# localdevices/pyorc

Measured on AMD Instinct MI355X. Metric: PIV frame-pairs/sec, 1080p 32x32@50% overlap (Mvectors/sec in config), higher is better.
Workload: dtype f32; 1 GPU; synthetic 1080x1920 uint8 particle stack, 1000 frame-pairs per GPU, 32x32 windows @ overlap 16 (BASELINE.json configs[1]); frame_dtype=u8, windows_per_pair=7854, parallelism=single GPU

## Files before the change

### pyorc_amd/csrc/api_internal.h

```cpp
#pragma once

#include "../../include/lspiv.h"

#include <hip/hip_runtime.h>

#include <atomic>
#include <cstdint>
#include <mutex>
#include <vector>

#include "common.h"
#include "host_stage.h"

namespace lspiv_api __attribute__((visibility("hidden"))) {

int fail(int code, const char* fmt, ...);

inline int hip_code(hipError_t e) {
  return e == hipErrorOutOfMemory ? LSPIV_ENOMEM : (e == hipErrorNoDevice || e == hipErrorNoBinaryForGpu) ? LSPIV_ENODEV : LSPIV_EHIP;
}

#define HIP_TRY(expr)                                                                                          \
  do {                                                                                                         \
    const hipError_t e_ = (expr);                                                                              \
    if (e_ != hipSuccess)                                                                                      \
      return fail(hip_code(e_), "%s failed: %s (%s:%d)", #expr, hipGetErrorString(e_), __FILE__, __LINE__);    \
  } while (0)

#define LSPIV_TRY(expr)                                                                        \
  do {                                                                                         \
    const int rc_ = (expr);                                                                    \
    if (rc_ != LSPIV_OK) return rc_;                                                           \
  } while (0)

inline int launch_status(hipError_t e, const char* what = "kernel launch failed", int oom_code = LSPIV_EHIP) {
  if (e == hipSuccess) return LSPIV_OK;
  return fail(e == hipErrorOutOfMemory ? oom_code : LSPIV_EHIP, "%s: %s", what, hipGetErrorString(e));
}

inline size_t elem_size(int dtype) { return dtype == LSPIV_U8 ? 1 : dtype == LSPIV_F32 ? 4 : 8; }

struct Grid {
  int64_t n_rows = 0, n_cols = 0;
};
int make_grid(int64_t H, int64_t W, int wy, int wx, int oy, int ox, Grid* g);

struct DeviceCtx {
  hipStream_t stream = nullptr;
  hipStream_t copy_stream = nullptr;
  void* d_frames = nullptr;  size_t frames_cap = 0;
  float* d_out = nullptr;    size_t out_cap = 0;
  float* d_planes = nullptr; size_t planes_cap = 0;
  void* d_scratch = nullptr; size_t scratch_cap = 0;
  void* d_dft = nullptr; size_t dft_cap = 0;
  uint8_t* d_keep = nullptr; size_t keep_cap = 0;
  struct RescueWs { hipStream_t stream; void* base; size_t cap_bytes; uint32_t cap_fit, cap_amb; };
  std::vector<RescueWs> rescue;
  void* pinned[2] = {nullptr, nullptr}; size_t pinned_cap = 0;
  hipEvent_t staged[2] = {nullptr, nullptr};
  struct ProjWs { hipStream_t stream = nullptr; void* d_in = nullptr; size_t in_cap = 0; void* d_out = nullptr; size_t out_cap = 0;
                  void* pin[2] = {nullptr, nullptr}; hipEvent_t ev[2] = {nullptr, nullptr}; };
  static constexpr size_t kProjPinBytes = (size_t)16 << 20;
  static constexpr int kProjSlots = 2;
  ProjWs proj[kProjSlots];
  bool arch_ok = false;
};
constexpr int kMaxDevices = 64;
struct DeviceLocks { std::mutex host, dispatch, lists, project[DeviceCtx::kProjSlots]; std::atomic<unsigned> next_project{0}; };
extern DeviceLocks g_locks[kMaxDevices];
int current_device_slot();
inline DeviceLocks& locks_here() { return g_locks[current_device_slot()]; }
int get_ctx(DeviceCtx** out);
inline hipStream_t on_stream(const DeviceCtx* c, void* stream) { return stream ? (hipStream_t)stream : c->stream; }
template <class Launch>
int launch_on(void* stream, Launch&& launch) {
  DeviceCtx* c;
  const int rc = get_ctx(&c);
  return rc ? rc : launch_status(launch(on_stream(c, stream)));
}

struct TraceRec { int kind; hipEvent_t e0, e1; };
struct Trace;
struct TraceSpan {
  Trace* t = nullptr; TraceRec r{};
  ~TraceSpan();
};
void trace_begin(TraceSpan* sp, int kind, hipStream_t s);
void trace_end(TraceSpan* sp, hipStream_t s);

// ... 73 lines not shown
```

### pyorc_amd/csrc/api_piv.hip

```cpp
#include "api_internal.h"

#include <algorithm>
#include <cmath>
#include <cstdlib>
#include <cstring>

namespace lspiv_api __attribute__((visibility("hidden"))) {

int check_window(int wy, int wx, int oy, int ox) {
  if (wy < 2 || wx < 2 || wy > LSPIV_MAX_WINDOW || wx > LSPIV_MAX_WINDOW)
    return fail(LSPIV_EUNSUPPORTED, "window %dx%d outside supported range 2..%d", wy, wx, LSPIV_MAX_WINDOW);
  if (oy < 0 || ox < 0 || oy >= wy || ox >= wx)
    return fail(LSPIV_EINVAL, "overlap (%d,%d) must satisfy 0 <= overlap < window (%d,%d)", oy, ox, wy, wx);
  return LSPIV_OK;
}

int64_t axis_shape(int64_t dim, int win, int ov) { return dim < win ? 0 : (dim - win) / (win - ov) + 1; }

int make_grid(int64_t H, int64_t W, int wy, int wx, int oy, int ox, Grid* g) {
  LSPIV_TRY(check_window(wy, wx, oy, ox));
  if (H <= 0 || W <= 0) return fail(LSPIV_ESHAPE, "frame shape (%lld,%lld) invalid", (long long)H, (long long)W);
  g->n_rows = axis_shape(H, wy, oy);
  g->n_cols = axis_shape(W, wx, ox);
  if (g->n_rows <= 0 || g->n_cols <= 0)
    return fail(LSPIV_ESHAPE, "frame (%lld,%lld) smaller than window (%d,%d)", (long long)H, (long long)W, wy, wx);
  return LSPIV_OK;
}

int rescue_ws(DeviceCtx* c, hipStream_t s, uint32_t n_tiles, lspiv::PivParams* p) {
  std::lock_guard<std::mutex> lk(locks_here().lists);
  DeviceCtx::RescueWs* ws = nullptr;
  for (auto& w : c->rescue) if (w.stream == s) ws = &w;
  if (!ws) { c->rescue.push_back({s, nullptr, 0, 0, 0}); ws = &c->rescue.back(); }
  const uint32_t cap_fit = std::max<uint32_t>(4096u, n_tiles / 4u), cap_amb = std::max<uint32_t>(1024u, n_tiles / 16u);
  const size_t hdr_bytes = 256;
  static_assert(sizeof(lspiv::RescueHdr) <= 256, "header slot too small");
  if (cap_fit > ws->cap_fit || cap_amb > ws->cap_amb || !ws->base) {
    const uint32_t nf = std::max(cap_fit, ws->cap_fit), na = std::max(cap_amb, ws->cap_amb);
    const size_t bytes = hdr_bytes + (size_t)nf * sizeof(uint4) + (size_t)na * sizeof(uint32_t);
    void* grown = nullptr;
    HIP_TRY(hipMalloc(&grown, bytes));
    if (ws->base) {
      hipError_t e = hipStreamSynchronize(s);
      if (e == hipSuccess) e = hipMemcpy(grown, ws->base, hdr_bytes, hipMemcpyDeviceToDevice);
      if (e != hipSuccess) { (void)hipFree(grown); return fail(LSPIV_EHIP, "rescue lists: %s", hipGetErrorString(e)); }
      HIP_TRY(hipFree(ws->base));
    } else {
      HIP_TRY(hipMemsetAsync(grown, 0, hdr_bytes, s));
    }
    ws->base = grown;
    ws->cap_bytes = bytes; ws->cap_fit = nf; ws->cap_amb = na;
  }
  p->rescue_hdr = static_cast<lspiv::RescueHdr*>(ws->base);
  p->rescue_fit = reinterpret_cast<uint4*>((char*)ws->base + hdr_bytes);
  p->rescue_amb = reinterpret_cast<uint32_t*>((char*)ws->base + hdr_bytes + (size_t)ws->cap_fit * sizeof(uint4));
  p->rescue_cap_fit = ws->cap_fit;
  p->rescue_cap_amb = ws->cap_amb;
  return LSPIV_OK;
}

int fill_params(lspiv::PivParams* p, const void* d_frames, int dtype, int64_t T, int64_t H, int64_t W, int wy, int wx,
                int oy, int ox, float signal_threshold, const Grid& g) {
  if (dtype < 0 || dtype > 2) return fail(LSPIV_EINVAL, "dtype %d not in {0:u8, 1:f32, 2:f64}", dtype);
  if (T < 2) return fail(LSPIV_ESHAPE, "need at least 2 frames, got %lld", (long long)T);
  const int64_t n_win = g.n_rows * g.n_cols;
  const int64_t n_tiles = (T - 1) * n_win;
  if (n_tiles >= (int64_t)1 << 31 || H * W >= (int64_t)1 << 31)
    return fail(LSPIV_EINVAL, "chunk too large for one launch: %lld windows (limit 2^31); use smaller chunks",
                (long long)n_tiles);
  memset(p, 0, sizeof(*p));
  p->frames = d_frames;
  p->frame_elems = H * W;
  p->H = (int)H; p->W = (int)W;
  p->wy = wy; p->wx = wx;
  p->sy = wy - oy; p->sx = wx - ox;
  p->n_rows = (int)g.n_rows; p->n_cols = (int)g.n_cols;
  p->n_win = (uint32_t)n_win;
  p->n_tiles = (uint32_t)n_tiles;
  p->n_pairs = (uint32_t)(T - 1);
  p->signal_threshold = signal_threshold;
  p->border_mode = g_opt_border.load();
  p->nz_positive = g_opt_signal_pos.load();
  {
    const double n = (double)wy * (double)wx;
    const double g2 = g_opt_std_ddof.load() && n > 1.0 ? (n - 1.0) / n : 1.0;
    p->std_gain2 = (float)g2;
// ... 4 lines not shown
  p->rescue_tau = (float)(g_opt_rescue_tau.load() * 1e-9);
  p->div_ncols = lspiv::FastDiv::make((uint32_t)g.n_cols);
  p->div_jobs = lspiv::FastDiv::make((uint32_t)((n_win + 1) / 2));
  p->div_nwin = lspiv::FastDiv::make((uint32_t)n_win);
  return LSPIV_OK;
}

static int dispatch_kernels(const lspiv::PivParams& p, int dtype, bool ensemble, hipStream_t s);

constexpr int kTimerRing = 16;
struct KernelTimer { hipEvent_t e0[kTimerRing] = {}, e1[kTimerRing] = {}; int n = 0; };
KernelTimer g_timers[kMaxDevices];
static int timed_dispatch_kernels(const lspiv::PivParams& p, int dtype, bool ensemble, hipStream_t s) {
  if (!g_opt_time_kernel.load()) return dispatch_kernels(p, dtype, ensemble, s);
  KernelTimer& t = g_timers[current_device_slot()];
  const int k = t.n % kTimerRing;
  if (!t.e0[k]) { HIP_TRY(hipEventCreate(&t.e0[k])); HIP_TRY(hipEventCreate(&t.e1[k])); }
  HIP_TRY(hipEventRecord(t.e0[k], s));
  LSPIV_TRY(dispatch_kernels(p, dtype, ensemble, s));
  HIP_TRY(hipEventRecord(t.e1[k], s));
  ++t.n;
  return LSPIV_OK;
}
int dispatch(const lspiv::PivParams& p0, int dtype, bool ensemble, hipStream_t s) {
  if (ensemble || !g_opt_rescue.load()) {
    if (!g_opt_time_kernel.load()) return dispatch_kernels(p0, dtype, ensemble, s);
    std::lock_guard<std::mutex> launch_lock(locks_here().dispatch);
    return timed_dispatch_kernels(p0, dtype, ensemble, s);
  }
  DeviceCtx* c;
  LSPIV_TRY(get_ctx(&c));
  lspiv::PivParams p = p0;
  std::lock_guard<std::mutex> launch_lock(locks_here().dispatch);
  LSPIV_TRY(rescue_ws(c, s, p.n_tiles, &p));
  LSPIV_TRY(timed_dispatch_kernels(p, dtype, false, s));
  return launch_status(lspiv::launch_piv_rescue(p, dtype, s), "rescue kernel launch failed");
}

int apply_v_sign(float* d_v, int64_t n, hipStream_t s) {
  if (!g_opt_v_sign.load() || !d_v) return LSPIV_OK;
  return launch_status(lspiv::launch_negate(d_v, n, s));
}

static int dispatch_kernels(const lspiv::PivParams& p, int dtype, bool ensemble, hipStream_t s) {
  const int kind = lspiv_kernel_kind(p.wy, p.wx);
  hipError_t e;
  switch (kind) {
    case 7: e = lspiv::launch_piv_embed16(p, dtype, ensemble, s); break;
    case 4: e = lspiv::launch_piv_embed32(p, dtype, ensemble, s); break;
    case 5: e = lspiv::launch_piv_embed64(p, dtype, ensemble, s); break;
    case 6: e = p.wy == 8 ? lspiv::launch_piv_fft8(p, dtype, ensemble, s) : lspiv::launch_piv_fft16(p, dtype, ensemble, s); break;
    case 8:
      switch (p.wy) {
#define LSPIV_PFA_CASE(n) case n: e = lspiv::launch_piv_fft##n(p, dtype, ensemble, s); break;
        LSPIV_PFA_SIZES(LSPIV_PFA_CASE)
#undef LSPIV_PFA_CASE
        default: return fail(LSPIV_EUNSUPPORTED, "no prime-factor kernel for window %d", p.wy);
      }
      break;
    case 1: e = lspiv::launch_piv_fft32(p, dtype, ensemble, s); break;
    case 2: e = lspiv::launch_piv_fft64(p, dtype, ensemble, s); break;
    case 3: e = lspiv::launch_piv_direct(p, dtype, ensemble, s); break;
    case 9: e = lspiv::launch_piv_dft(p, dtype, ensemble, s); break;
    case 10: {
      DeviceCtx* c;
      LSPIV_TRY(get_ctx(&c));
      const size_t slot = lspiv::piv_dft_global_slot_floats(p.wy, p.wx);
      const int blocks = lspiv::piv_dft_global_blocks(ensemble ? p.n_win : p.n_tiles);
      LSPIV_TRY(ensure(&c->d_dft, &c->dft_cap, slot * (size_t)blocks * sizeof(float)));
// ... 310 lines not shown
```

### pyorc_amd/csrc/common.h

```cpp
#pragma once
#include <hip/hip_runtime.h>
#include <stdint.h>

#include <algorithm>

namespace lspiv {

struct FastDiv {
  uint32_t magic, shift, d;
  static __host__ FastDiv make(uint32_t d) {
    FastDiv f;
    f.d = d;
    uint32_t l = 31;
    while (l > 0 && !((d >> l) & 1u)) --l;
    if ((d & (d - 1)) == 0) {
      f.magic = 0;
      f.shift = l == 0 ? 0 : l - 1;
      return f;
    }
    const uint64_t num = (uint64_t)1 << (32 + l);
    uint64_t m = num / d;
    const uint64_t rem = num - m * d;
    m += m;
    const uint64_t twice_rem = rem + rem;
    if (twice_rem >= d) m += 1;
    f.magic = (uint32_t)(m + 1);
    f.shift = l;
    return f;
  }
  __host__ __device__ __forceinline__ uint32_t div(uint32_t n) const {
    if (d == 1) return n;
#ifdef __HIP_DEVICE_COMPILE__
    const uint32_t q = __umulhi(magic, n);
#else
    const uint32_t q = (uint32_t)(((uint64_t)magic * n) >> 32);
#endif
    return (((n - q) >> 1) + q) >> shift;
  }
};

struct RescueHdr {
  uint32_t n_fit, n_amb;
  uint32_t spare0, spare1;
  uint32_t done_blocks, pad;
  uint32_t last_fit, last_amb;
  unsigned long long total_fit, total_amb, total_windows;
};

struct PivParams {
  const void* frames;
  int64_t frame_elems;
  int H, W;
  int wy, wx;
  int sy, sx;
  int n_rows, n_cols;
  uint32_t n_win;
  uint32_t n_tiles;
  float signal_threshold;
  int border_mode;
  int nz_positive;
  const uint8_t* win_keep;
  float std_gain, std_gain2;
  int norm_clip;
  float* u;
  float* v;
  float* cmax;
  float* s2n;
  float* planes;
  float corr_min, s2n_min;
  float* corr_sum;
  float* corr_count;
  float* part_sum;
  float* part_cnt;
  float* dft_scratch;
  size_t dft_slot;
  uint32_t seg_len, n_seg;
  uint32_t seg_first;
// ... 215 lines not shown
__device__ __forceinline__ void rescue_note(RescueHdr* hdr, uint4* fit, uint32_t cap_fit, uint32_t* amb, uint32_t cap_amb,
                                            uint32_t g, PeakCond c, int ip, int jp, uint32_t pos2 = 0xffffffffu) {
  if (c.amb && pos2 == 0xffffffffu) {
    const uint32_t i = atomicAdd(&hdr->n_amb, 1u);
    if (i < cap_amb) amb[i] = g;
  } else if (c.amb || c.fit) {
    const uint32_t i = atomicAdd(&hdr->n_fit, 1u);
    if (i < cap_fit) fit[i] = make_uint4(g, ((uint32_t)ip << 16) | (uint32_t)jp, pos2, 0u);
  }
}

__device__ __forceinline__ float to_f32(uint8_t x) { return (float)x; }
__device__ __forceinline__ float to_f32(float x) { return x; }
__device__ __forceinline__ float to_f32(double x) { return (float)x; }

hipError_t launch_piv_fft8(const PivParams& p, int dtype, bool ensemble, hipStream_t s);
hipError_t launch_piv_fft16(const PivParams& p, int dtype, bool ensemble, hipStream_t s);
#define LSPIV_PFA_SIZES(X) X(6) X(10) X(12) X(14) X(18) X(20) X(22) X(24) X(26) X(28) X(30) X(34) X(36) X(38) X(40) X(42) X(44) X(46) \
  X(48) X(50) X(52) X(54) X(56) X(58) X(60) X(62)
#define LSPIV_PFA_DECL(n) hipError_t launch_piv_fft##n(const PivParams& p, int dtype, bool ensemble, hipStream_t s);
LSPIV_PFA_SIZES(LSPIV_PFA_DECL)
#undef LSPIV_PFA_DECL
hipError_t launch_piv_fft32(const PivParams& p, int dtype, bool ensemble, hipStream_t s);
hipError_t launch_piv_fft64(const PivParams& p, int dtype, bool ensemble, hipStream_t s);
hipError_t launch_piv_direct(const PivParams& p, int dtype, bool ensemble, hipStream_t s);
hipError_t launch_piv_dft(const PivParams& p, int dtype, bool ensemble, hipStream_t s);
bool piv_dft_fits(int wy, int wx);
size_t piv_dft_global_slot_floats(int wy, int wx);
int piv_dft_global_blocks(uint32_t n_work);
hipError_t launch_piv_dft_global(const PivParams& p, int dtype, bool ensemble, hipStream_t s);
hipError_t launch_piv_embed16(const PivParams& p, int dtype, bool ensemble, hipStream_t s);
hipError_t launch_piv_embed32(const PivParams& p, int dtype, bool ensemble, hipStream_t s);
hipError_t launch_piv_embed64(const PivParams& p, int dtype, bool ensemble, hipStream_t s);
hipError_t launch_piv_rescue(const PivParams& p, int dtype, hipStream_t s);
hipError_t launch_ens_flag(const float* mean, uint32_t n_win, int wy, int wx, const float* u, const float* v, float k, float tau,
                           EnsRescueHdr* hdr, EnsRescueRec* recs, uint32_t cap, hipStream_t s);
hipError_t launch_ens_partial(const PivParams& p, int dtype, const EnsRescueArgs& a, hipStream_t s);
hipError_t launch_ens_merge(const EnsRescueArgs& a, double* totals, hipStream_t s);
hipError_t launch_ens_final(const PivParams& p, const EnsRescueArgs& a, const double* totals, float* u, float* v, hipStream_t s);
hipError_t launch_peaks_from_planes(const float* planes, uint32_t n_planes, int wy, int wx, int border_mode,
                                    float* u, float* v, hipStream_t s);
hipError_t launch_window_signal(const void* frames, int dtype, int64_t T, const PivParams& p, float thr, uint8_t* keep, hipStream_t s);
int walk_setting();
constexpr uint32_t kWalkAnchor = 25;
constexpr uint32_t kWalkAnchorLong = 75;
inline uint32_t walk_long_min_windows(int n) {
  return n <= 16 ? 256u * 4u * 3u * 4u : n <= 32 ? 256u * 4u * 3u * 2u : 256u * 4u * 2u;
}
inline uint32_t walk_anchor(int n, uint32_t n_win) { return n_win >= walk_long_min_windows(n) ? kWalkAnchorLong : kWalkAnchor; }
struct WalkSegments { uint32_t seg_len, seg_first, n_seg; };
inline WalkSegments walk_segments(uint32_t n_pairs, int64_t pair_offset, uint32_t seg_len) {
  WalkSegments w;
  w.seg_len = seg_len < 1 ? 1 : seg_len;
  const uint32_t head = (uint32_t)(pair_offset % (int64_t)w.seg_len);
  w.seg_first = std::min<uint32_t>(w.seg_len - head, n_pairs);
  w.n_seg = 1 + (n_pairs - w.seg_first + w.seg_len - 1) / w.seg_len;
  return w;
}
uint32_t job_slots(int waves_per_simd, int groups);
hipError_t launch_ensemble_merge(const float* part_sum, const float* part_cnt, uint32_t n_seg, uint32_t n_win, int plane_elems,
                                 float* corr_sum, float* corr_count, hipStream_t s, int lane_major_n = 0, bool split_halves = false);
hipError_t launch_ensemble_mean(const float* sum, const float* count, float min_count, uint32_t n_win,
                                int plane_elems, float* mean, hipStream_t s);
hipError_t launch_project(const void* frames, int dtype, int64_t src_elems, int n_frames, const int* nn_src,
                          const int* grp_of, const int* grp_off, const int* grp_src, float* out, int n_out,
                          hipStream_t s);
hipError_t launch_division_check(int* d_mismatches, hipStream_t s);
// ... 40 lines not shown
```

### pyorc_amd/csrc/piv_rescue.hip

```cpp
#include "common.h"

namespace lspiv {

namespace {

constexpr int RBLOCK = 256;
constexpr int RESCUE_LDS_SAMPLES = 4096;
constexpr int RESCUE_GENERIC_MAX = 16384;

template <int CTRL>
__device__ __forceinline__ double dpp_d(double x) {
  const unsigned long long b = __builtin_bit_cast(unsigned long long, x);
  const unsigned lo = (unsigned)dpp_i<CTRL>((int)(unsigned)b), hi = (unsigned)dpp_i<CTRL>((int)(unsigned)(b >> 32));
  return __builtin_bit_cast(double, ((unsigned long long)hi << 32) | lo);
}
__device__ __forceinline__ double wave_sum_d(double x) {
  x += dpp_d<DPP_XOR1>(x);
  x += dpp_d<DPP_XOR2>(x);
  x += dpp_d<DPP_HALF_MIRROR>(x);
  x += dpp_d<DPP_MIRROR>(x);
  {
    const unsigned long long b = __builtin_bit_cast(unsigned long long, x);
    const unsigned lo = (unsigned)swz16_i((int)(unsigned)b), hi = (unsigned)swz16_i((int)(unsigned)(b >> 32));
    x += __builtin_bit_cast(double, ((unsigned long long)hi << 32) | lo);
  }
  {
    const unsigned long long b = __builtin_bit_cast(unsigned long long, x);
    unsigned lo_a = (unsigned)b, lo_b = lo_a, hi_a = (unsigned)(b >> 32), hi_b = hi_a;
    permlane32_swap(lo_a, lo_b);
    permlane32_swap(hi_a, hi_b);
    x = __builtin_bit_cast(double, ((unsigned long long)hi_a << 32) | lo_a) + __builtin_bit_cast(double, ((unsigned long long)hi_b << 32) | lo_b);
  }
  return x;
}

struct LaneWalk {
  int qy, qx, wx;
  __device__ LaneWalk(int wx_) : qy(64 / wx_), qx(64 - (64 / wx_) * wx_), wx(wx_) {}
  __device__ __forceinline__ void start(int lane, int& y, int& x) const { y = lane / wx; x = lane - y * wx; }
  __device__ __forceinline__ void next(int& y, int& x) const {
    y += qy; x += qx;
    if (x >= wx) { x -= wx; ++y; }
  }
};

template <typename T, bool STAGE = false>
__device__ __forceinline__ void window_stats_wave2(const T* A, const T* B, int W, int wy, int wx, int lane, double& mean_a,
                                                   double& sd_a, double& mean_b, double& sd_b, T* la = nullptr, T* lb = nullptr) {
  const int n = wy * wx;
  const LaneWalk lw(wx);
  const double x0a = (double)A[0], x0b = (double)B[0];
  double sa = 0.0, sb = 0.0, qa = 0.0, qb = 0.0;
  int y, x;
  lw.start(lane, y, x);
#pragma unroll 8
  for (int e = lane; e < n; e += 64, lw.next(y, x)) {
    const int64_t off = (int64_t)y * W + x;
    const T ra = A[off], rb = B[off];
    if constexpr (STAGE) { la[e] = ra; lb[e] = rb; }
    const double da = (double)ra - x0a, db = (double)rb - x0b;
    sa += da; qa = fma(da, da, qa);
    sb += db; qb = fma(db, db, qb);
  }
  sa = wave_sum_d(sa); sb = wave_sum_d(sb); qa = wave_sum_d(qa); qb = wave_sum_d(qb);
  const double inv_n = 1.0 / (double)n;
  mean_a = x0a + sa * inv_n;
  mean_b = x0b + sb * inv_n;
  const double va = (qa - sa * sa * inv_n) * inv_n, vb = (qb - sb * sb * inv_n) * inv_n;
  sd_a = va > 0.0 ? sqrt(va) : 0.0;
  sd_b = vb > 0.0 ? sqrt(vb) : 0.0;
}

__device__ __forceinline__ double norm_clip(double x, double mean, double inv_sd) {
  const double d = (x - mean) * fabs(inv_sd);
  return (d > 0.0 || inv_sd < 0.0) ? d : 0.0;
}

__device__ __forceinline__ int unshift(int ip, int c, int w) { return ip - c < 0 ? ip - c + w : ip - c; }

template <typename PA>
__device__ __forceinline__ uint32_t choose_wave(const PivParams& p, PA A, PA B, int pitch, double mean_a, double inv_a, double mean_b,
                                                double inv_b, uint32_t pos1, uint32_t pos2, int lane) {
  const int wy = p.wy, wx = p.wx, n = wy * wx, cy = wy / 2, cx = wx / 2;
  const int ky1 = unshift((int)(pos1 >> 16), cy, wy), kx1 = unshift((int)(pos1 & 0xffffu), cx, wx);
  const int ky2 = unshift((int)(pos2 >> 16), cy, wy), kx2 = unshift((int)(pos2 & 0xffffu), cx, wx);
  const LaneWalk lw(wx);
  double acc1 = 0.0, acc2 = 0.0;
  int y, x;
  lw.start(lane, y, x);
#pragma unroll 4
  for (int e = lane; e < n; e += 64, lw.next(y, x)) {
    const double av = norm_clip((double)A[y * pitch + x], mean_a, inv_a);
    int y1 = y + ky1; y1 = y1 >= wy ? y1 - wy : y1;
    int x1 = x + kx1; x1 = x1 >= wx ? x1 - wx : x1;
    int y2 = y + ky2; y2 = y2 >= wy ? y2 - wy : y2;
    int x2 = x + kx2; x2 = x2 >= wx ? x2 - wx : x2;
    acc1 += av * norm_clip((double)B[y1 * pitch + x1], mean_b, inv_b);
    acc2 += av * norm_clip((double)B[y2 * pitch + x2], mean_b, inv_b);
  }
  const double c1 = wave_sum_d(acc1), c2 = wave_sum_d(acc2);
  const uint32_t o1 = (pos1 >> 16) * (uint32_t)wx + (pos1 & 0xffffu), o2 = (pos2 >> 16) * (uint32_t)wx + (pos2 & 0xffffu);
  return (c2 > c1 || (c2 == c1 && o2 < o1)) ? pos2 : pos1;
}

struct Lag5 { double c0, cu, cd, cl, cr; };
template <typename PA>
__device__ __forceinline__ Lag5 lag5_wave(const PivParams& p, PA A, PA B, int pitch, double mean_a, double inv_a, double mean_b,
                                          double inv_b, int ip, int jp, int lane) {
  const int wy = p.wy, wx = p.wx, n = wy * wx, cy = wy / 2, cx = wx / 2;
  const int ky0 = unshift(ip, cy, wy), kx0 = unshift(jp, cx, wx);
  const int kym = ky0 == 0 ? wy - 1 : ky0 - 1, kyp = ky0 == wy - 1 ? 0 : ky0 + 1;
  const int kxm = kx0 == 0 ? wx - 1 : kx0 - 1, kxp = kx0 == wx - 1 ? 0 : kx0 + 1;
  const LaneWalk lw(wx);
  double acc0 = 0.0, accu = 0.0, accd = 0.0, accl = 0.0, accr = 0.0;
  int y, x;
  lw.start(lane, y, x);
#pragma unroll 4
  for (int e = lane; e < n; e += 64, lw.next(y, x)) {
    const double av = norm_clip((double)A[y * pitch + x], mean_a, inv_a);
    int y0 = y + ky0; y0 = y0 >= wy ? y0 - wy : y0;
    int ym = y + kym; ym = ym >= wy ? ym - wy : ym;
    int yp = y + kyp; yp = yp >= wy ? yp - wy : yp;
    int x0 = x + kx0; x0 = x0 >= wx ? x0 - wx : x0;
    int xm = x + kxm; xm = xm >= wx ? xm - wx : xm;
    int xp = x + kxp; xp = xp >= wx ? xp - wx : xp;
    acc0 += av * norm_clip((double)B[y0 * pitch + x0], mean_b, inv_b);
    accu += av * norm_clip((double)B[ym * pitch + x0], mean_b, inv_b);
    accd += av * norm_clip((double)B[yp * pitch + x0], mean_b, inv_b);
    accl += av * norm_clip((double)B[y0 * pitch + xm], mean_b, inv_b);
    accr += av * norm_clip((double)B[y0 * pitch + xp], mean_b, inv_b);
  }
  const double inv_n = 1.0 / (double)n;
  auto clip01 = [](double c) { return c < 0.0 ? 0.0 : (c > 1.0 ? 1.0 : c); };
  Lag5 o;
  o.c0 = clip01(wave_sum_d(acc0) * inv_n); o.cu = clip01(wave_sum_d(accu) * inv_n); o.cd = clip01(wave_sum_d(accd) * inv_n);
  o.cl = clip01(wave_sum_d(accl) * inv_n); o.cr = clip01(wave_sum_d(accr) * inv_n);
  return o;
}
__device__ __forceinline__ void fit5_d(const Lag5& c, int ip, int jp, int cy, int cx, float& u, float& v) {
  const double eps = 1e-7;
  const double l0 = log(c.c0 + eps), lu = log(c.cu + eps), ld = log(c.cd + eps), ll = log(c.cl + eps), lr = log(c.cr + eps);
  const double den1 = 2 * lu - 4 * l0 + 2 * ld, den2 = 2 * ll - 4 * l0 + 2 * lr;
  const double di = den1 != 0.0 ? (lu - ld) / den1 : 0.0;
  const double dj = den2 != 0.0 ? (ll - lr) / den2 : 0.0;
  v = (float)((double)ip + di - (double)cy);
  u = (float)((double)jp + dj - (double)cx);
}

template <typename PA>
__device__ __forceinline__ void fit_wave(const PivParams& p, PA A, PA B, int pitch, double mean_a, double inv_a, double mean_b,
                                         double inv_b, uint32_t g, int ip, int jp, int lane) {
  const int wy = p.wy, wx = p.wx, cy = wy / 2, cx = wx / 2;
  if (ip <= 0 || ip >= wy - 1 || jp <= 0 || jp >= wx - 1) {
    if (lane == 0) {
      float u, v;
      border_result(p.border_mode, jp - cx, ip - cy, u, v);
      p.u[g] = u; p.v[g] = v;
    }
    return;
  }
  const Lag5 c = lag5_wave(p, A, B, pitch, mean_a, inv_a, mean_b, inv_b, ip, jp, lane);
  const double eps = 1e-7;
  const double mine = log((lane == 0 ? c.c0 : lane == 1 ? c.cu : lane == 2 ? c.cd : lane == 3 ? c.cl : c.cr) + eps);
  const double l0 = __shfl(mine, 0, 64), lu = __shfl(mine, 1, 64), ld = __shfl(mine, 2, 64), ll = __shfl(mine, 3, 64), lr = __shfl(mine, 4, 64);
  if (lane == 0) {
    const double den1 = 2 * lu - 4 * l0 + 2 * ld, den2 = 2 * ll - 4 * l0 + 2 * lr;
    const double di = den1 != 0.0 ? (lu - ld) / den1 : 0.0;
    const double dj = den2 != 0.0 ? (ll - lr) / den2 : 0.0;
    p.v[g] = (float)((double)ip + di - (double)cy);
    p.u[g] = (float)((double)jp + dj - (double)cx);
  }
}

template <typename T>
__device__ __forceinline__ const T* window_base(const PivParams& p, uint32_t g) {
  const uint32_t pair = g / p.n_win, win = g - pair * p.n_win;
  const uint32_t wrow = win / (uint32_t)p.n_cols, wcol = win - wrow * (uint32_t)p.n_cols;
  return static_cast<const T*>(p.frames) + ((int64_t)pair * p.H + (int64_t)wrow * p.sy) * p.W + (int64_t)wcol * p.sx;
}

__device__ __forceinline__ void amax_merge_d(double& v, int& idx, double pv, int pidx) {
  const bool take = (pv > v) || (pv == v && pidx < idx);
  v = take ? pv : v;
  idx = take ? pidx : idx;
}

constexpr int FIT_LDS_PER_WAVE = 8192;

template <typename T>
__global__ __launch_bounds__(RBLOCK) void piv_rescue_fit_kernel(PivParams p) {
  extern __shared__ __attribute__((aligned(16))) unsigned char fsm[];
  typedef const T __attribute__((address_space(3))) * LdsPtr;
  const RescueHdr* hdr = p.rescue_hdr;
  const int lane = threadIdx.x & 63, wave = threadIdx.x >> 6;
  const int wy = p.wy, wx = p.wx, n = wy * wx;
  const bool staged = (size_t)2 * n * sizeof(T) <= (size_t)FIT_LDS_PER_WAVE;
  T* la = reinterpret_cast<T*>(fsm + (size_t)wave * FIT_LDS_PER_WAVE);
  T* lb = la + n;
  const uint32_t n_fit = min(hdr->n_fit, p.rescue_cap_fit);
  const uint32_t n_waves = gridDim.x * (RBLOCK / 64);
  for (uint32_t i = blockIdx.x * (RBLOCK / 64) + (uint32_t)wave; i < n_fit; i += n_waves) {
    const uint4 rec = p.rescue_fit[i];
    const uint32_t g = rec.x;
    if (g >= p.n_tiles) continue;
    const T* A = window_base<T>(p, g);
    const T* B = A + p.frame_elems;
    double mean_a, sd_a, mean_b, sd_b;
    if (staged) window_stats_wave2<T, true>(A, B, p.W, wy, wx, lane, mean_a, sd_a, mean_b, sd_b, la, lb);
    else window_stats_wave2<T, false>(A, B, p.W, wy, wx, lane, mean_a, sd_a, mean_b, sd_b, nullptr, nullptr);
    if (sd_a != 0.0 && sd_b != 0.0) {
      const double sg = p.norm_clip ? (double)p.std_gain : -(double)p.std_gain;
      const double inv_a = sg / sd_a, inv_b = sg / sd_b;
      uint32_t pos = rec.y;
      if (staged) {
        __builtin_amdgcn_wave_barrier();
        const LdsPtr SA = (LdsPtr)la, SB = (LdsPtr)lb;
        if (rec.z != 0xffffffffu) pos = choose_wave(p, SA, SB, wx, mean_a, inv_a, mean_b, inv_b, rec.y, rec.z, lane);
        fit_wave(p, SA, SB, wx, mean_a, inv_a, mean_b, inv_b, g, (int)(pos >> 16), (int)(pos & 0xffffu), lane);
        __builtin_amdgcn_wave_barrier();
      } else {
        if (rec.z != 0xffffffffu) pos = choose_wave(p, A, B, p.W, mean_a, inv_a, mean_b, inv_b, rec.y, rec.z, lane);
        fit_wave(p, A, B, p.W, mean_a, inv_a, mean_b, inv_b, g, (int)(pos >> 16), (int)(pos & 0xffffu), lane);
      }
    }
  }
}

constexpr int AMB_R = 4;

template <typename T>
__global__ __launch_bounds__(RBLOCK) void piv_rescue_amb_kernel(PivParams p) {
  extern __shared__ __attribute__((aligned(16))) double dsm[];
  __shared__ double red_v[RBLOCK / 64];
  __shared__ int red_i[RBLOCK / 64];
  RescueHdr* hdr = p.rescue_hdr;
  const int lane = threadIdx.x & 63, wave = threadIdx.x >> 6;
  const int wy = p.wy, wx = p.wx, n = wy * wx, cy = wy / 2, cx = wx / 2;
  const uint32_t n_amb = min(hdr->n_amb, p.rescue_cap_amb);
  const bool fast = n <= RESCUE_LDS_SAMPLES && (wx % AMB_R) == 0;
  const int pitch = 2 * wx;
  double* la = dsm;
  double* lb2 = dsm + n;
  int* lx = reinterpret_cast<int*>(dsm + 3 * n);
  int* lcnt = lx + n;
  for (uint32_t i = blockIdx.x; i < n_amb; i += gridDim.x) {
    __syncthreads();
    const uint32_t g = min(p.rescue_amb[i], p.n_tiles - 1);
    const bool g_ok = p.rescue_amb[i] < p.n_tiles;
    const T* A = window_base<T>(p, g);
    const T* B = A + p.frame_elems;
    double mean_a, sd_a, mean_b, sd_b;
    window_stats_wave2<T>(A, B, p.W, wy, wx, lane, mean_a, sd_a, mean_b, sd_b);
    const bool dead = sd_a == 0.0 || sd_b == 0.0;
    const double sg = p.norm_clip ? (double)p.std_gain : -(double)p.std_gain;
    const double inv_a = dead ? 1.0 : sg / sd_a, inv_b = dead ? 1.0 : sg / sd_b;
    double best = -1.0;
    int bi = 0x7fffffff;
    if (fast) {
      for (int e = threadIdx.x; e < n; e += RBLOCK) {
        const int y = e / wx, x = e - y * wx;
        la[e] = norm_clip((double)A[(int64_t)y * p.W + x], mean_a, inv_a);
        const double bv = norm_clip((double)B[(int64_t)y * p.W + x], mean_b, inv_b);
        lb2[y * pitch + x] = bv;
        lb2[y * pitch + wx + x] = bv;
      }
      __syncthreads();
      for (int r = threadIdx.x; r < wy; r += RBLOCK) {
        double* ar = la + r * wx;
        int* xr = lx + r * wx;
        int k = 0;
        for (int x = 0; x < wx; ++x) {
          const double av = ar[x];
          if (av != 0.0) { ar[k] = av; xr[k] = x; ++k; }
        }
        lcnt[r] = k;
      }
      __syncthreads();
      const int strips_per_row = wx / AMB_R, strips = wy * strips_per_row;
// ... 30 lines not shown
    } else if (n <= RESCUE_GENERIC_MAX) {
      for (int o = threadIdx.x; o < n; o += RBLOCK) {
        const int ipo = o / wx, jpo = o - ipo * wx;
        const int ky = ipo - cy < 0 ? ipo - cy + wy : ipo - cy, kx = jpo - cx < 0 ? jpo - cx + wx : jpo - cx;
        double acc = 0.0;
        int yb = ky;
        for (int y = 0; y < wy; ++y) {
          int xb = kx;
          for (int x = 0; x < wx; ++x) {
            const double av = norm_clip((double)A[(int64_t)y * p.W + x], mean_a, inv_a);
            if (av != 0.0) acc += av * norm_clip((double)B[(int64_t)yb * p.W + xb], mean_b, inv_b);
            xb = xb + 1 == wx ? 0 : xb + 1;
          }
          yb = yb + 1 == wy ? 0 : yb + 1;
        }
        double c = acc / (double)n;
        c = c < 0.0 ? 0.0 : (c > 1.0 ? 1.0 : c);
        amax_merge_d(best, bi, c, o);
      }
    }
#pragma unroll
    for (int o = 32; o >= 1; o >>= 1) amax_merge_d(best, bi, __shfl_xor(best, o, 64), __shfl_xor(bi, o, 64));
    if (lane == 0) { red_v[wave] = best; red_i[wave] = bi; }
    __syncthreads();
    best = red_v[0]; bi = red_i[0];
#pragma unroll
    for (int k = 1; k < RBLOCK / 64; ++k) amax_merge_d(best, bi, red_v[k], red_i[k]);
    if (wave == 0 && !dead && g_ok && (fast || n <= RESCUE_GENERIC_MAX)) {
      const int ip = bi / wx, jp = bi - ip * wx;
      fit_wave(p, A, B, p.W, mean_a, inv_a, mean_b, inv_b, g, ip, jp, lane);
    }
  }

  __syncthreads();
  if (threadIdx.x == 0) {
    __threadfence();
    const uint32_t d = atomicAdd(&hdr->done_blocks, 1u);
    if (d == gridDim.x - 1) {
      hdr->last_fit = hdr->n_fit;
      hdr->last_amb = hdr->n_amb;
      hdr->total_fit += hdr->n_fit;
      hdr->total_amb += hdr->n_amb;
      hdr->total_windows += p.n_tiles;
      hdr->n_fit = 0; hdr->n_amb = 0; hdr->done_blocks = 0;
      __threadfence();
    }
  }
}

__device__ __forceinline__ void wave_argmax_first(float& v, int& idx) {
#pragma unroll
  for (int o = 32; o >= 1; o >>= 1) {
    const float pv = __shfl_xor(v, o, 64);
    const int pi = __shfl_xor(idx, o, 64);
    const bool take = (pv > v) || (pv == v && pi < idx);
    v = take ? pv : v;
    idx = take ? pi : idx;
  }
}
__device__ __forceinline__ int wave_min_i(int x) {
#pragma unroll
  for (int o = 32; o >= 1; o >>= 1) x = min(x, __shfl_xor(x, o, 64));
  return x;
}
__device__ __forceinline__ int wave_sum_i(int x) {
#pragma unroll
  for (int o = 32; o >= 1; o >>= 1) x += __shfl_xor(x, o, 64);
  return x;
}

__global__ __launch_bounds__(RBLOCK) void ens_flag_kernel(const float* mean, uint32_t n_win, int wy, int wx, const float* u, const float* v,
                                                          float k, float tau, EnsRescueHdr* hdr, EnsRescueRec* recs, uint32_t cap) {
  const int lane = threadIdx.x & 63;
  const uint32_t w = blockIdx.x * (RBLOCK / 64) + (threadIdx.x >> 6);
  if (w >= n_win) return;
  const int n = wy * wx;
  const float* pl = mean + (size_t)w * n;
  float best = -1.0f;
  int bi = 0x7fffffff;
// ... 100 lines not shown
  const uint32_t i = blockIdx.x * RBLOCK + threadIdx.x;
  if (i >= a.n_rec * ROW) return;
  const uint32_t ri = i / ROW, q = i - ri * ROW;
  const double* src = a.partial + (size_t)ri * a.n_blk * ROW + q;
  double sum = 0.0;
  for (uint32_t b = 0; b < a.n_blk; ++b) sum += src[(size_t)b * ROW];
  totals[i] = sum;
}

__global__ __launch_bounds__(RBLOCK) void ens_final_kernel(PivParams p, EnsRescueArgs a, const double* totals, float* u, float* v) {
  constexpr int ROW = kEnsMaxCand * 5;
  const uint32_t ri = blockIdx.x * RBLOCK + threadIdx.x;
  if (ri >= a.n_rec) return;
  const EnsRescueRec rec = a.recs[ri];
  if (rec.ncand == 0) return;
  const double cnt = (double)a.count[rec.w];
  if (!(cnt > 0.0)) return;
  const int cy = p.wy / 2, cx = p.wx / 2;
  int best = -1;
  Lag5 bl = {0, 0, 0, 0, 0};
  for (int c = 0; c < (int)rec.ncand; ++c) {
    const double* t = totals + (size_t)ri * ROW + c * 5;
    const Lag5 l = {t[0] / cnt, t[1] / cnt, t[2] / cnt, t[3] / cnt, t[4] / cnt};
    if (best < 0 || l.c0 > bl.c0) { best = c; bl = l; }
  }
  const int ip = (int)(rec.pos[best] >> 16), jp = (int)(rec.pos[best] & 0xffffu);
  float uu, vv;
  if (ip <= 0 || ip >= p.wy - 1 || jp <= 0 || jp >= p.wx - 1) border_result(p.border_mode, jp - cx, ip - cy, uu, vv);
  else fit5_d(bl, ip, jp, cy, cx, uu, vv);
  u[rec.w] = uu; v[rec.w] = vv;
}

template <typename T>
hipError_t launch_rescue_t(const PivParams& p, hipStream_t s) {
  const int n = p.wy * p.wx;
  const bool fast = n <= RESCUE_LDS_SAMPLES && (p.wx % AMB_R) == 0;
  const size_t lds = fast ? (size_t)3 * n * sizeof(double) + (size_t)(n + p.wy) * sizeof(int) : 0;
  const uint32_t fit_blocks = std::min<uint32_t>(4096u, std::max<uint32_t>(64u, p.n_tiles / 512u + 1u));
  const uint32_t amb_blocks = std::min<uint32_t>(1024u, std::max<uint32_t>(64u, p.n_tiles / 2048u + 1u));
  const size_t fit_lds = (size_t)2 * n * sizeof(T) <= (size_t)FIT_LDS_PER_WAVE ? (size_t)(RBLOCK / 64) * FIT_LDS_PER_WAVE : 0;
  hipLaunchKernelGGL(piv_rescue_fit_kernel<T>, dim3(fit_blocks), dim3(RBLOCK), fit_lds, s, p);
  hipError_t e = hipGetLastError();
  if (e != hipSuccess) return e;
  e = hipFuncSetAttribute(reinterpret_cast<const void*>(&piv_rescue_amb_kernel<T>), hipFuncAttributeMaxDynamicSharedMemorySize,
                          (int)(3 * RESCUE_LDS_SAMPLES * sizeof(double) + (RESCUE_LDS_SAMPLES + 512) * sizeof(int)));
  if (e != hipSuccess) return e;
  hipLaunchKernelGGL(piv_rescue_amb_kernel<T>, dim3(amb_blocks), dim3(RBLOCK), lds, s, p);
  return hipGetLastError();
}

}

hipError_t launch_ens_flag(const float* mean, uint32_t n_win, int wy, int wx, const float* u, const float* v, float k, float tau,
                           EnsRescueHdr* hdr, EnsRescueRec* recs, uint32_t cap, hipStream_t s) {
  if (n_win == 0) return hipSuccess;
  hipLaunchKernelGGL(ens_flag_kernel, dim3((n_win + RBLOCK / 64 - 1) / (RBLOCK / 64)), dim3(RBLOCK), 0, s, mean, n_win, wy, wx, u, v, k, tau,
                     hdr, recs, cap);
  return hipGetLastError();
}

template <typename T>
static void launch_ens_partial_t(const PivParams& p, const EnsRescueArgs& a, uint32_t blocks, hipStream_t s) {
  const int n = p.wy * p.wx;
  const size_t lds = (size_t)2 * n * sizeof(T) <= (size_t)FIT_LDS_PER_WAVE ? (size_t)(RBLOCK / 64) * FIT_LDS_PER_WAVE : 0;
  hipLaunchKernelGGL(ens_partial_kernel<T>, dim3(blocks), dim3(RBLOCK), lds, s, p, a);
}

hipError_t launch_ens_partial(const PivParams& p, int dtype, const EnsRescueArgs& a, hipStream_t s) {
  const uint32_t chunk_blks = (a.n_pairs + kEnsPairBlock - 1) / kEnsPairBlock;
  const uint64_t items = (uint64_t)a.n_rec * chunk_blks;
  if (items == 0) return hipSuccess;
  const uint32_t blocks = (uint32_t)std::min<uint64_t>((items + RBLOCK / 64 - 1) / (RBLOCK / 64), 65536);
  switch (dtype) {
    case 0: launch_ens_partial_t<uint8_t>(p, a, blocks, s); break;
    case 1: launch_ens_partial_t<float>(p, a, blocks, s); break;
    case 2: launch_ens_partial_t<double>(p, a, blocks, s); break;
    default: return hipErrorInvalidValue;
  }
  return hipGetLastError();
}

hipError_t launch_ens_merge(const EnsRescueArgs& a, double* totals, hipStream_t s) {
  if (a.n_rec == 0) return hipSuccess;
  const uint32_t n = a.n_rec * kEnsMaxCand * 5;
  hipLaunchKernelGGL(ens_merge_kernel, dim3((n + RBLOCK - 1) / RBLOCK), dim3(RBLOCK), 0, s, a, totals);
  return hipGetLastError();
}

hipError_t launch_ens_final(const PivParams& p, const EnsRescueArgs& a, const double* totals, float* u, float* v, hipStream_t s) {
  if (a.n_rec == 0) return hipSuccess;
  hipLaunchKernelGGL(ens_final_kernel, dim3((a.n_rec + RBLOCK - 1) / RBLOCK), dim3(RBLOCK), 0, s, p, a, totals, u, v);
  return hipGetLastError();
}

hipError_t launch_piv_rescue(const PivParams& p, int dtype, hipStream_t s) {
  if (!p.rescue_hdr) return hipSuccess;
  switch (dtype) {
    case 0: return launch_rescue_t<uint8_t>(p, s);
    case 1: return launch_rescue_t<float>(p, s);
    case 2: return launch_rescue_t<double>(p, s);
    default: return hipErrorInvalidValue;
  }
}

}
```

Measured before the change: 151,700 frame-pairs/s.

## Fuse rescue fit and ambiguity kernels into one launch with double-buffered header

Merges the separate rescue fit and ambiguity kernels into a single launch, split by block index. The last-block atomic counter that reset the header is replaced by a two-slot header that alternates per pass, and block 0 records the stats. The fit path also stages pre-normalised B samples as doubles in LDS, so the per-lag normalisation is not recomputed. This removes one kernel launch and the completion atomic and fences, at the cost of more LDS per block and a shared launch shape for two different workloads.

```diff
diff --git a/pyorc_amd/csrc/api_internal.h b/pyorc_amd/csrc/api_internal.h
--- a/pyorc_amd/csrc/api_internal.h
+++ b/pyorc_amd/csrc/api_internal.h
@@ -54,7 +54,7 @@
   void* d_scratch = nullptr; size_t scratch_cap = 0;
   void* d_dft = nullptr; size_t dft_cap = 0;
   uint8_t* d_keep = nullptr; size_t keep_cap = 0;
-  struct RescueWs { hipStream_t stream; void* base; size_t cap_bytes; uint32_t cap_fit, cap_amb; };
+  struct RescueWs { hipStream_t stream; void* base; size_t cap_bytes; uint32_t cap_fit, cap_amb; uint64_t passes; };
   std::vector<RescueWs> rescue;
   void* pinned[2] = {nullptr, nullptr}; size_t pinned_cap = 0;
   hipEvent_t staged[2] = {nullptr, nullptr};
diff --git a/pyorc_amd/csrc/api_piv.hip b/pyorc_amd/csrc/api_piv.hip
--- a/pyorc_amd/csrc/api_piv.hip
+++ b/pyorc_amd/csrc/api_piv.hip
@@ -27,14 +27,14 @@
   return LSPIV_OK;
 }
 
-int rescue_ws(DeviceCtx* c, hipStream_t s, uint32_t n_tiles, lspiv::PivParams* p) {
+int rescue_ws(DeviceCtx* c, hipStream_t s, uint32_t n_tiles, lspiv::PivParams* p, lspiv::RescueHdr** stats, lspiv::RescueHdr** next) {
   std::lock_guard<std::mutex> lk(locks_here().lists);
   DeviceCtx::RescueWs* ws = nullptr;
   for (auto& w : c->rescue) if (w.stream == s) ws = &w;
-  if (!ws) { c->rescue.push_back({s, nullptr, 0, 0, 0}); ws = &c->rescue.back(); }
+  if (!ws) { c->rescue.push_back({s, nullptr, 0, 0, 0, 0}); ws = &c->rescue.back(); }
   const uint32_t cap_fit = std::max<uint32_t>(4096u, n_tiles / 4u), cap_amb = std::max<uint32_t>(1024u, n_tiles / 16u);
   const size_t hdr_bytes = 256;
-  static_assert(sizeof(lspiv::RescueHdr) <= 256, "header slot too small");
+  static_assert(sizeof(lspiv::RescueHdr) <= 128, "header slot too small");
   if (cap_fit > ws->cap_fit || cap_amb > ws->cap_amb || !ws->base) {
     const uint32_t nf = std::max(cap_fit, ws->cap_fit), na = std::max(cap_amb, ws->cap_amb);
     const size_t bytes = hdr_bytes + (size_t)nf * sizeof(uint4) + (size_t)na * sizeof(uint32_t);
@@ -51,7 +51,11 @@
     ws->base = grown;
     ws->cap_bytes = bytes; ws->cap_fit = nf; ws->cap_amb = na;
   }
-  p->rescue_hdr = static_cast<lspiv::RescueHdr*>(ws->base);
+  lspiv::RescueHdr* slot[2] = {static_cast<lspiv::RescueHdr*>(ws->base), reinterpret_cast<lspiv::RescueHdr*>((char*)ws->base + 128)};
+  p->rescue_hdr = slot[ws->passes & 1];
+  *next = slot[(ws->passes + 1) & 1];
+  *stats = slot[0];
+  ++ws->passes;
   p->rescue_fit = reinterpret_cast<uint4*>((char*)ws->base + hdr_bytes);
   p->rescue_amb = reinterpret_cast<uint32_t*>((char*)ws->base + hdr_bytes + (size_t)ws->cap_fit * sizeof(uint4));
   p->rescue_cap_fit = ws->cap_fit;
@@ -122,9 +126,10 @@
   LSPIV_TRY(get_ctx(&c));
   lspiv::PivParams p = p0;
   std::lock_guard<std::mutex> launch_lock(locks_here().dispatch);
-  LSPIV_TRY(rescue_ws(c, s, p.n_tiles, &p));
+  lspiv::RescueHdr *stats, *next;
+  LSPIV_TRY(rescue_ws(c, s, p.n_tiles, &p, &stats, &next));
   LSPIV_TRY(timed_dispatch_kernels(p, dtype, false, s));
-  return launch_status(lspiv::launch_piv_rescue(p, dtype, s), "rescue kernel launch failed");
+  return launch_status(lspiv::launch_piv_rescue(p, stats, next, dtype, s), "rescue kernel launch failed");
 }
 
 int apply_v_sign(float* d_v, int64_t n, hipStream_t s) {
diff --git a/pyorc_amd/csrc/common.h b/pyorc_amd/csrc/common.h
--- a/pyorc_amd/csrc/common.h
+++ b/pyorc_amd/csrc/common.h
@@ -42,7 +42,7 @@
 struct RescueHdr {
   uint32_t n_fit, n_amb;
   uint32_t spare0, spare1;
-  uint32_t done_blocks, pad;
+  uint32_t spare2, pad;
   uint32_t last_fit, last_amb;
   unsigned long long total_fit, total_amb, total_windows;
 };
@@ -324,7 +324,7 @@
 hipError_t launch_piv_embed16(const PivParams& p, int dtype, bool ensemble, hipStream_t s);
 hipError_t launch_piv_embed32(const PivParams& p, int dtype, bool ensemble, hipStream_t s);
 hipError_t launch_piv_embed64(const PivParams& p, int dtype, bool ensemble, hipStream_t s);
-hipError_t launch_piv_rescue(const PivParams& p, int dtype, hipStream_t s);
+hipError_t launch_piv_rescue(const PivParams& p, RescueHdr* stats, RescueHdr* next, int dtype, hipStream_t s);
 hipError_t launch_ens_flag(const float* mean, uint32_t n_win, int wy, int wx, const float* u, const float* v, float k, float tau,
                            EnsRescueHdr* hdr, EnsRescueRec* recs, uint32_t cap, hipStream_t s);
 hipError_t launch_ens_partial(const PivParams& p, int dtype, const EnsRescueArgs& a, hipStream_t s);
diff --git a/pyorc_amd/csrc/piv_rescue.hip b/pyorc_amd/csrc/piv_rescue.hip
--- a/pyorc_amd/csrc/piv_rescue.hip
+++ b/pyorc_amd/csrc/piv_rescue.hip
@@ -44,7 +44,7 @@
   }
 };
 
-template <typename T, bool STAGE = false>
+template <typename T, bool STAGE = false, bool STAGE_B = STAGE>
 __device__ __forceinline__ void window_stats_wave2(const T* A, const T* B, int W, int wy, int wx, int lane, double& mean_a,
                                                    double& sd_a, double& mean_b, double& sd_b, T* la = nullptr, T* lb = nullptr) {
   const int n = wy * wx;
@@ -57,7 +57,10 @@
   for (int e = lane; e < n; e += 64, lw.next(y, x)) {
     const int64_t off = (int64_t)y * W + x;
     const T ra = A[off], rb = B[off];
-    if constexpr (STAGE) { la[e] = ra; lb[e] = rb; }
+    if constexpr (STAGE) {
+      la[e] = ra;
+      if constexpr (STAGE_B) lb[e] = rb;
+    }
     const double da = (double)ra - x0a, db = (double)rb - x0b;
     sa += da; qa = fma(da, da, qa);
     sb += db; qb = fma(db, db, qb);
@@ -76,10 +79,15 @@
   return (d > 0.0 || inv_sd < 0.0) ? d : 0.0;
 }
 
+struct NormSample { double v; };
+template <typename PB>
+__device__ __forceinline__ double norm_at(PB B, int idx, double mean, double inv_sd) { return norm_clip((double)B[idx], mean, inv_sd); }
+__device__ __forceinline__ double norm_at(const NormSample __attribute__((address_space(3))) * B, int idx, double, double) { return B[idx].v; }
+
 __device__ __forceinline__ int unshift(int ip, int c, int w) { return ip - c < 0 ? ip - c + w : ip - c; }
 
-template <typename PA>
-__device__ __forceinline__ uint32_t choose_wave(const PivParams& p, PA A, PA B, int pitch, double mean_a, double inv_a, double mean_b,
+template <typename PA, typename PB>
+__device__ __forceinline__ uint32_t choose_wave(const PivParams& p, PA A, PB B, int pitch, double mean_a, double inv_a, double mean_b,
                                                 double inv_b, uint32_t pos1, uint32_t pos2, int lane) {
   const int wy = p.wy, wx = p.wx, n = wy * wx, cy = wy / 2, cx = wx / 2;
   const int ky1 = unshift((int)(pos1 >> 16), cy, wy), kx1 = unshift((int)(pos1 & 0xffffu), cx, wx);
@@ -95,8 +103,8 @@
     int x1 = x + kx1; x1 = x1 >= wx ? x1 - wx : x1;
     int y2 = y + ky2; y2 = y2 >= wy ? y2 - wy : y2;
     int x2 = x + kx2; x2 = x2 >= wx ? x2 - wx : x2;
-    acc1 += av * norm_clip((double)B[y1 * pitch + x1], mean_b, inv_b);
-    acc2 += av * norm_clip((double)B[y2 * pitch + x2], mean_b, inv_b);
+    acc1 += av * norm_at(B, y1 * pitch + x1, mean_b, inv_b);
+    acc2 += av * norm_at(B, y2 * pitch + x2, mean_b, inv_b);
   }
   const double c1 = wave_sum_d(acc1), c2 = wave_sum_d(acc2);
   const uint32_t o1 = (pos1 >> 16) * (uint32_t)wx + (pos1 & 0xffffu), o2 = (pos2 >> 16) * (uint32_t)wx + (pos2 & 0xffffu);
@@ -104,8 +112,8 @@
 }
 
 struct Lag5 { double c0, cu, cd, cl, cr; };
-template <typename PA>
-__device__ __forceinline__ Lag5 lag5_wave(const PivParams& p, PA A, PA B, int pitch, double mean_a, double inv_a, double mean_b,
+template <typename PA, typename PB>
+__device__ __forceinline__ Lag5 lag5_wave(const PivParams& p, PA A, PB B, int pitch, double mean_a, double inv_a, double mean_b,
                                           double inv_b, int ip, int jp, int lane) {
   const int wy = p.wy, wx = p.wx, n = wy * wx, cy = wy / 2, cx = wx / 2;
   const int ky0 = unshift(ip, cy, wy), kx0 = unshift(jp, cx, wx);
@@ -124,11 +132,11 @@
     int x0 = x + kx0; x0 = x0 >= wx ? x0 - wx : x0;
     int xm = x + kxm; xm = xm >= wx ? xm - wx : xm;
     int xp = x + kxp; xp = xp >= wx ? xp - wx : xp;
-    acc0 += av * norm_clip((double)B[y0 * pitch + x0], mean_b, inv_b);
-    accu += av * norm_clip((double)B[ym * pitch + x0], mean_b, inv_b);
-    accd += av * norm_clip((double)B[yp * pitch + x0], mean_b, inv_b);
-    accl += av * norm_clip((double)B[y0 * pitch + xm], mean_b, inv_b);
-    accr += av * norm_clip((double)B[y0 * pitch + xp], mean_b, inv_b);
+    acc0 += av * norm_at(B, y0 * pitch + x0, mean_b, inv_b);
+    accu += av * norm_at(B, ym * pitch + x0, mean_b, inv_b);
+    accd += av * norm_at(B, yp * pitch + x0, mean_b, inv_b);
+    accl += av * norm_at(B, y0 * pitch + xm, mean_b, inv_b);
+    accr += av * norm_at(B, y0 * pitch + xp, mean_b, inv_b);
   }
   const double inv_n = 1.0 / (double)n;
   auto clip01 = [](double c) { return c < 0.0 ? 0.0 : (c > 1.0 ? 1.0 : c); };
@@ -147,8 +155,8 @@
   u = (float)((double)jp + dj - (double)cx);
 }
 
-template <typename PA>
-__device__ __forceinline__ void fit_wave(const PivParams& p, PA A, PA B, int pitch, double mean_a, double inv_a, double mean_b,
+template <typename PA, typename PB>
+__device__ __forceinline__ void fit_wave(const PivParams& p, PA A, PB B, int pitch, double mean_a, double inv_a, double mean_b,
                                          double inv_b, uint32_t g, int ip, int jp, int lane) {
   const int wy = p.wy, wx = p.wx, cy = wy / 2, cx = wx / 2;
   if (ip <= 0 || ip >= wy - 1 || jp <= 0 || jp >= wx - 1) {
@@ -187,32 +195,50 @@
 
 constexpr int FIT_LDS_PER_WAVE = 8192;
 
+constexpr int NORM_LDS_PER_WAVE = 9216;
+
 template <typename T>
-__global__ __launch_bounds__(RBLOCK) void piv_rescue_fit_kernel(PivParams p) {
+__device__ __forceinline__ void rescue_fit_part(const PivParams& p, uint32_t blk, uint32_t n_blk) {
   extern __shared__ __attribute__((aligned(16))) unsigned char fsm[];
   typedef const T __attribute__((address_space(3))) * LdsPtr;
+  typedef const NormSample __attribute__((address_space(3))) * LdsNorm;
   const RescueHdr* hdr = p.rescue_hdr;
-  const int lane = threadIdx.x & 63, wave = threadIdx.x >> 6;
+  const int lane = threadIdx.x & 63, wave = __builtin_amdgcn_readfirstlane(threadIdx.x >> 6);
   const int wy = p.wy, wx = p.wx, n = wy * wx;
+  const bool norm = (size_t)n * (sizeof(double) + sizeof(T)) <= (size_t)NORM_LDS_PER_WAVE;
   const bool staged = (size_t)2 * n * sizeof(T) <= (size_t)FIT_LDS_PER_WAVE;
-  T* la = reinterpret_cast<T*>(fsm + (size_t)wave * FIT_LDS_PER_WAVE);
+  double* lbn = reinterpret_cast<double*>(fsm + (size_t)wave * NORM_LDS_PER_WAVE);
+  T* la = norm ? reinterpret_cast<T*>(lbn + n) : reinterpret_cast<T*>(fsm + (size_t)wave * FIT_LDS_PER_WAVE);
   T* lb = la + n;
   const uint32_t n_fit = min(hdr->n_fit, p.rescue_cap_fit);
-  const uint32_t n_waves = gridDim.x * (RBLOCK / 64);
-  for (uint32_t i = blockIdx.x * (RBLOCK / 64) + (uint32_t)wave; i < n_fit; i += n_waves) {
+  const uint32_t n_waves = n_blk * (RBLOCK / 64);
+  for (uint32_t i = blk * (RBLOCK / 64) + (uint32_t)wave; i < n_fit; i += n_waves) {
     const uint4 rec = p.rescue_fit[i];
     const uint32_t g = rec.x;
     if (g >= p.n_tiles) continue;
     const T* A = window_base<T>(p, g);
     const T* B = A + p.frame_elems;
     double mean_a, sd_a, mean_b, sd_b;
-    if (staged) window_stats_wave2<T, true>(A, B, p.W, wy, wx, lane, mean_a, sd_a, mean_b, sd_b, la, lb);
+    if (norm) window_stats_wave2<T, true, false>(A, B, p.W, wy, wx, lane, mean_a, sd_a, mean_b, sd_b, la, nullptr);
+    else if (staged) window_stats_wave2<T, true>(A, B, p.W, wy, wx, lane, mean_a, sd_a, mean_b, sd_b, la, lb);
     else window_stats_wave2<T, false>(A, B, p.W, wy, wx, lane, mean_a, sd_a, mean_b, sd_b, nullptr, nullptr);
     if (sd_a != 0.0 && sd_b != 0.0) {
       const double sg = p.norm_clip ? (double)p.std_gain : -(double)p.std_gain;
       const double inv_a = sg / sd_a, inv_b = sg / sd_b;
       uint32_t pos = rec.y;
-      if (staged) {
+      if (norm) {
+        const LaneWalk lw(wx);
+        int y, x;
+        lw.start(lane, y, x);
+#pragma unroll 8
+        for (int e = lane; e < n; e += 64, lw.next(y, x)) lbn[e] = norm_clip((double)B[(int64_t)y * p.W + x], mean_b, inv_b);
+        __builtin_amdgcn_wave_barrier();
+        const LdsPtr SA = (LdsPtr)la;
+        const LdsNorm SB = (LdsNorm)lbn;
+        if (rec.z != 0xffffffffu) pos = choose_wave(p, SA, SB, wx, mean_a, inv_a, mean_b, inv_b, rec.y, rec.z, lane);
+        fit_wave(p, SA, SB, wx, mean_a, inv_a, mean_b, inv_b, g, (int)(pos >> 16), (int)(pos & 0xffffu), lane);
+        __builtin_amdgcn_wave_barrier();
+      } else if (staged) {
         __builtin_amdgcn_wave_barrier();
         const LdsPtr SA = (LdsPtr)la, SB = (LdsPtr)lb;
         if (rec.z != 0xffffffffu) pos = choose_wave(p, SA, SB, wx, mean_a, inv_a, mean_b, inv_b, rec.y, rec.z, lane);
@@ -229,11 +255,11 @@
 constexpr int AMB_R = 4;
 
 template <typename T>
-__global__ __launch_bounds__(RBLOCK) void piv_rescue_amb_kernel(PivParams p) {
+__device__ __forceinline__ void rescue_amb_part(const PivParams& p, uint32_t blk, uint32_t n_blk) {
   extern __shared__ __attribute__((aligned(16))) double dsm[];
   __shared__ double red_v[RBLOCK / 64];
   __shared__ int red_i[RBLOCK / 64];
-  RescueHdr* hdr = p.rescue_hdr;
+  const RescueHdr* hdr = p.rescue_hdr;
   const int lane = threadIdx.x & 63, wave = threadIdx.x >> 6;
   const int wy = p.wy, wx = p.wx, n = wy * wx, cy = wy / 2, cx = wx / 2;
   const uint32_t n_amb = min(hdr->n_amb, p.rescue_cap_amb);
@@ -243,7 +269,7 @@
   double* lb2 = dsm + n;
   int* lx = reinterpret_cast<int*>(dsm + 3 * n);
   int* lcnt = lx + n;
-  for (uint32_t i = blockIdx.x; i < n_amb; i += gridDim.x) {
+  for (uint32_t i = blk; i < n_amb; i += n_blk) {
     __syncthreads();
     const uint32_t g = min(p.rescue_amb[i], p.n_tiles - 1);
     const bool g_ok = p.rescue_amb[i] < p.n_tiles;
@@ -340,19 +366,20 @@
     }
   }
 
-  __syncthreads();
-  if (threadIdx.x == 0) {
-    __threadfence();
-    const uint32_t d = atomicAdd(&hdr->done_blocks, 1u);
-    if (d == gridDim.x - 1) {
-      hdr->last_fit = hdr->n_fit;
-      hdr->last_amb = hdr->n_amb;
-      hdr->total_fit += hdr->n_fit;
-      hdr->total_amb += hdr->n_amb;
-      hdr->total_windows += p.n_tiles;
-      hdr->n_fit = 0; hdr->n_amb = 0; hdr->done_blocks = 0;
-      __threadfence();
-    }
+}
+
+template <typename T>
+__global__ __launch_bounds__(RBLOCK) void piv_rescue_kernel(PivParams p, RescueHdr* stats, RescueHdr* next, uint32_t amb_blocks) {
+  if (blockIdx.x < amb_blocks) rescue_amb_part<T>(p, blockIdx.x, amb_blocks);
+  else rescue_fit_part<T>(p, blockIdx.x - amb_blocks, gridDim.x - amb_blocks);
+  if (blockIdx.x == 0 && threadIdx.x == 0) {
+    const RescueHdr* cur = p.rescue_hdr;
+    stats->last_fit = cur->n_fit;
+    stats->last_amb = cur->n_amb;
+    stats->total_fit += cur->n_fit;
+    stats->total_amb += cur->n_amb;
+    stats->total_windows += p.n_tiles;
+    next->n_fit = 0; next->n_amb = 0;
   }
 }
 
@@ -519,20 +546,20 @@
 }
 
 template <typename T>
-hipError_t launch_rescue_t(const PivParams& p, hipStream_t s) {
+hipError_t launch_rescue_t(const PivParams& p, RescueHdr* stats, RescueHdr* next, hipStream_t s) {
   const int n = p.wy * p.wx;
   const bool fast = n <= RESCUE_LDS_SAMPLES && (p.wx % AMB_R) == 0;
-  const size_t lds = fast ? (size_t)3 * n * sizeof(double) + (size_t)(n + p.wy) * sizeof(int) : 0;
+  const size_t amb_lds = fast ? (size_t)3 * n * sizeof(double) + (size_t)(n + p.wy) * sizeof(int) : 0;
   const uint32_t fit_blocks = std::min<uint32_t>(4096u, std::max<uint32_t>(64u, p.n_tiles / 512u + 1u));
   const uint32_t amb_blocks = std::min<uint32_t>(1024u, std::max<uint32_t>(64u, p.n_tiles / 2048u + 1u));
-  const size_t fit_lds = (size_t)2 * n * sizeof(T) <= (size_t)FIT_LDS_PER_WAVE ? (size_t)(RBLOCK / 64) * FIT_LDS_PER_WAVE : 0;
-  hipLaunchKernelGGL(piv_rescue_fit_kernel<T>, dim3(fit_blocks), dim3(RBLOCK), fit_lds, s, p);
-  hipError_t e = hipGetLastError();
+  const size_t fit_lds = (size_t)n * (sizeof(double) + sizeof(T)) <= (size_t)NORM_LDS_PER_WAVE ? (size_t)(RBLOCK / 64) * NORM_LDS_PER_WAVE
+                        : (size_t)2 * n * sizeof(T) <= (size_t)FIT_LDS_PER_WAVE       ? (size_t)(RBLOCK / 64) * FIT_LDS_PER_WAVE
+                                                                                       : 0;
+  hipError_t e = hipFuncSetAttribute(reinterpret_cast<const void*>(&piv_rescue_kernel<T>), hipFuncAttributeMaxDynamicSharedMemorySize,
+                                     (int)(3 * RESCUE_LDS_SAMPLES * sizeof(double) + (RESCUE_LDS_SAMPLES + 512) * sizeof(int)));
   if (e != hipSuccess) return e;
-  e = hipFuncSetAttribute(reinterpret_cast<const void*>(&piv_rescue_amb_kernel<T>), hipFuncAttributeMaxDynamicSharedMemorySize,
-                          (int)(3 * RESCUE_LDS_SAMPLES * sizeof(double) + (RESCUE_LDS_SAMPLES + 512) * sizeof(int)));
-  if (e != hipSuccess) return e;
-  hipLaunchKernelGGL(piv_rescue_amb_kernel<T>, dim3(amb_blocks), dim3(RBLOCK), lds, s, p);
+  hipLaunchKernelGGL(piv_rescue_kernel<T>, dim3(amb_blocks + fit_blocks), dim3(RBLOCK), std::max(amb_lds, fit_lds), s, p, stats, next,
+                     amb_blocks);
   return hipGetLastError();
 }
 
@@ -580,12 +607,12 @@
   return hipGetLastError();
 }
 
-hipError_t launch_piv_rescue(const PivParams& p, int dtype, hipStream_t s) {
+hipError_t launch_piv_rescue(const PivParams& p, RescueHdr* stats, RescueHdr* next, int dtype, hipStream_t s) {
   if (!p.rescue_hdr) return hipSuccess;
   switch (dtype) {
-    case 0: return launch_rescue_t<uint8_t>(p, s);
-    case 1: return launch_rescue_t<float>(p, s);
-    case 2: return launch_rescue_t<double>(p, s);
+    case 0: return launch_rescue_t<uint8_t>(p, stats, next, s);
+    case 1: return launch_rescue_t<float>(p, stats, next, s);
+    case 2: return launch_rescue_t<double>(p, stats, next, s);
     default: return hipErrorInvalidValue;
   }
 }
```

Result: no change. 152,400 frame-pairs/s (median of 6 runs) (+0.5%).
